# wenyuqing/panacea

Hardware: AMD Instinct MI355X
Metric: denoising steps/s (6-view x 8-frame 256x512) (higher is better)
Workload: dtype f16; 1 GPU; BASELINE config 3: Panacea+ stage-2 UNet+ControlNet, CFG 2 x 8 frames, 6 views, latent 32x384, hint 256x3072, Euler/LegacyDDPM 50-step schedule; precision=precise: split(stream,gn_stt,ff_out,stem,gn_head,gnt)+e4m3-lo, parallelism=single, graph=False, streams=2, hoisted_step_invariants=False, fused_step_tail=True

## Files before the change

### include/panacea_hip.h

```cpp
#ifndef PANACEA_HIP_H
#define PANACEA_HIP_H

#include <stdint.h>

#ifdef __cplusplus
extern "C" {
#endif

#define PNC_OK 0
#define PNC_EINVAL (-1)
#define PNC_EALIGN (-2)
#define PNC_EABI (-3)

const char* pnc_version(void);
#define PNC_ABI_VERSION 8
int pnc_abi_version(void);
const char* pnc_build_digest(void);

enum {
    PNC_OPT_GEMM_TAIL_SPLIT = 0,
    PNC_OPT_GEMM_TILE = 1,
    PNC_OPT_ATTN_VARIANT = 2,
    PNC_OPT_ATTN_DMA = 3,
    PNC_OPT_GEMM_FUSE_LN = 4,
    PNC_OPT_GEMM_GROUP_M = 5,
    PNC_OPT_STENCIL_TILES = 6,
    PNC_OPT_GEMM_PERSIST = 7,
    PNC_OPT_ATTN_DEFER_MAX = 8,
    PNC_OPT_GEMM_GN_STATS = 9,
    PNC_OPT_GEMM_STAGGER = 10,
    PNC_OPT_ATTN_SUM_TRIGGER = 11,
    PNC_OPT_COUNT = 12
};
int pnc_set_option(int option, int value);

enum { PNC_A_PLAIN = 0, PNC_A_CONV3X3 = 1, PNC_A_CONV1D_T = 2 };
enum { PNC_LO_F16 = 0, PNC_LO_E4M3 = 1 };
enum { PNC_ACT_NONE = 0, PNC_ACT_SILU = 1, PNC_ACT_GELU = 2  };

typedef struct PncGemmParams {
    const void* A;
    const void* W;
    int32_t M, N, K;
    int32_t lda;
    int32_t a_mode;
// ... 44 lines not shown
    int32_t groups;
    int32_t heads;
    int32_t H, W, views;
    int32_t kvH, kvW, kv_views;
    int32_t kv_rows_per_group;
    int32_t q_per_kv;
    int32_t kv_valid;
    int32_t nseg[8];
    int32_t seg[8][2];
    float scale;
    int32_t causal;
    const void* k_halo[2];
    const void* vt_halo[2];
} PncAttnParams;

int pnc_attn_views_f16(const PncAttnParams* p, void* stream);

int pnc_attn_temporal_f16(const void* q, int ldq, const void* k, int ldk,
                          const void* v, int ldv, void* o, int ldo,
                          int B, int T, int Npix, int heads, float scale, void* stream);

typedef struct PncAttnSplitParams {
    int32_t struct_bytes;
    PncAttnParams a;
    const void* q_lo;
    const void* k_lo;
    const void* v_lo;
    void* o_lo;
} PncAttnSplitParams;
int pnc_attn_views_split_f16(const PncAttnSplitParams* p, void* stream);
int pnc_attn_temporal_split_f16(const void* q, const void* q_lo, int ldq, const void* k, const void* k_lo, int ldk,
                                const void* v, const void* v_lo, int ldv, void* o, void* o_lo, int ldo,
                                int B, int T, int Npix, int heads, float scale, void* stream);

int pnc_groupnorm_stats(const float* x, int ldx, int F, int Npix, int C,
                        int pix_per_chunk, float* partial, void* stream);
int pnc_groupnorm_apply(const float* x, int ldx, int F, int Npix, int C,
                        int pix_per_chunk, const float* partial,
                        const float* gamma, const float* beta, float eps, int silu,
                        void* y16, int ldy, void* y16_lo, int lo_fmt, int n_records, void* stream);
int pnc_groupnorm_combine(const float* in, int parts, int F, int nchunk, float* out, void* stream);
int pnc_groupnorm_temporal_silu(const float* x, int B, int T, int Npix, int C,
                                const float* gamma, const float* beta, float eps,
                                void* y16, void* y16_lo, int lo_fmt, void* stream);
int pnc_groupnorm_temporal_part(const float* x, int B, int T, int Npix, int C,
                                const float* gamma, const float* beta, float eps,
                                float* stats, int mode, int T_total,
                                void* y16, void* y16_lo, int lo_fmt, int t_pad, void* stream);
int pnc_layernorm(const float* x, int ldx, int M, int C,
                  const float* gamma, const float* beta, float eps,
                  void* y16, int ldy, void* y16_lo, void* stream);

int pnc_linear_smallm(const float* a, int lda, const void* W, const float* bias,
                      float* out, int ldo, int M, int N, int K, int silu_in, int silu_out,
                      void* stream);
#define PNC_SMALLM_MAX_SEGS 64
int pnc_linear_smallm_segments(const float* a, int lda, const void* W, const float* bias, float* out, int M,
                               int m0, int Mtot, int N, int K, const int32_t* seg_start, int nseg, int silu_in,
                               int silu_out, void* stream);
int pnc_timestep_embedding(const int64_t* t, int F, int dim, const float* freqs,
                           float* out, void* stream);
int pnc_nchw_to_tokens_f16(const float* a, int C1, const float* a_scale, int a_frames, const float* b, int C2,
                           int F, int Npix, int Cpad, void* out16, void* out16_lo, void* stream);
int pnc_cfg_euler_step(const float* eps_tok, int ld, int T, int Npix, int C, int cfg, float scale,
                       const float* x, const float* c_out, const float* sigma, const float* sigma_next, float* x_next,
                       void* stream);
// ... 44 lines not shown
```

### panacea_amd/build.py

```python
from __future__ import annotations

import hashlib
import os
import shutil
import subprocess
import sys
from pathlib import Path

PKG = Path(__file__).resolve().parent
ROOT = PKG.parent
CSRC = PKG / "csrc"
LIBDIR = PKG / "lib"
LIB = LIBDIR / "libpanacea_hip.so"
SOURCES = ["gemm.hip", "gemm_plain.hip", "gemm_conv3x3.hip", "gemm_stencil_tile.hip", "gemm_conv1d.hip", "attn.hip", "attn_split.hip", "norm.hip", "misc.hip"]
HEADERS = [CSRC / "common.h", CSRC / "gemm_kernel.h", ROOT / "include" / "panacea_hip.h"]
FLAGS = ["--offload-arch=gfx950", "-O3", "-std=c++17", "-fPIC", "-Wall", "-Wno-unused-function",
         "-I", str(ROOT / "include"), "-I", str(CSRC)]


def _hipcc() -> str:
    for cand in (os.environ.get("HIPCC"), shutil.which("hipcc"), "/opt/rocm/bin/hipcc"):
        if cand and Path(cand).exists():
            return cand
    raise RuntimeError("hipcc not found (expected /opt/rocm/bin/hipcc)")


def _digest() -> str:
    h = hashlib.sha256()
    for f in [CSRC / s for s in SOURCES] + HEADERS:
        h.update(f.read_bytes())
    h.update(" ".join(f.replace(str(ROOT), "<root>") for f in FLAGS).encode())
    return h.hexdigest()


def library_digest(lib: Path = LIB):
    try:
        blob = Path(lib).read_bytes()
    except OSError:
        return None
    i = blob.find(_DIGEST_MARK)
    if i < 0:
        return None
    j = blob.find(b"\0", i)
    return blob[i + len(_DIGEST_MARK):j].decode(errors="replace")


_DIGEST_MARK = b"pnc-build-digest:"
# ... 40 lines not shown
```

### panacea_amd/csrc/attn.hip

```cpp
#include "common.h"
#include <stdlib.h>

namespace {

constexpr int KT = 64;

__device__ __forceinline__ int kperm(int i) { return 16 * ((i >> 2) & 1) + 4 * (i >> 3) + (i & 3); }

__device__ __attribute__((aligned(16))) half_t g_attn_zero_chunk[8];

template <int NW, int QB, bool DMA>
__global__ __launch_bounds__(64 * NW, (NW == 4 && QB == 2 && DMA) ? 2 : 1) void attn_views_kernel(const PncAttnParams p, const int wv_shift,
                                                                                          const float defer_thr, const int dma_mode,
                                                                                          const float sum_lim) {
    constexpr int QT = NW * QB * 32;
    constexpr int ROWS_PER_IT = NW * 8;
    constexpr int ST_IT = 64 / ROWS_PER_IT;
    constexpr int NST = DMA ? 3 : 2;
    __shared__ __attribute__((aligned(16))) char smem[NST * 2 * KT * 128];
    const half_t* __restrict__ Q = reinterpret_cast<const half_t*>(p.q);
    const half_t* __restrict__ K = reinterpret_cast<const half_t*>(p.k);
    const half_t* __restrict__ VT = reinterpret_cast<const half_t*>(p.vt);
    half_t* __restrict__ O = reinterpret_cast<half_t*>(p.o);
    auto seg_view = [&](int id, const half_t*& Kb, const half_t*& Vb) -> int {
// ... 534 lines not shown
extern "C" int pnc_attn_views_f16(const PncAttnParams* pp, void* stream) {
    if (!pp) return PNC_EINVAL;
    const PncAttnParams& p = *pp;
    if (!p.q || !p.k || !p.vt || !p.o) return PNC_EINVAL;
    if (p.views < 1 || p.views > 8 || p.kv_views < 1 || p.kv_views > 8) return PNC_EINVAL;
    if (p.W % p.views || p.kvW % p.kv_views) return PNC_EINVAL;
    const int kvWv = p.kvW / p.kv_views;
    (void)kvWv;
    if (p.ldq % 8 || p.ldk % 8 || p.ldo % 4) return PNC_EALIGN;
    if (((uintptr_t)p.q | (uintptr_t)p.k) & 15) return PNC_EALIGN;
    if ((uintptr_t)p.vt & 15) return PNC_EALIGN;
    if ((uintptr_t)p.o & 7) return PNC_EALIGN;
    if (p.q_per_kv < 1 || p.groups < 1 || p.heads < 1) return PNC_EINVAL;
    if (p.kv_valid < 1 || p.kv_valid > p.kvH * kvWv) return PNC_EINVAL;
    if (p.causal != 0 && p.causal != 1) return PNC_EINVAL;
    for (int v = 0; v < p.views; ++v) {
        if (p.nseg[v] < 1 || p.nseg[v] > 2) return PNC_EINVAL;
        for (int s = 0; s < p.nseg[v]; ++s) {
            const int id = p.seg[v][s];
            if (id == -1 || id == p.kv_views) {
                const int side = id < 0 ? 0 : 1;
                if (!p.k_halo[side] || !p.vt_halo[side]) return PNC_EINVAL;
                if (((uintptr_t)p.k_halo[side] | (uintptr_t)p.vt_halo[side]) & 15) return PNC_EALIGN;
            } else if (id < 0 || id > p.kv_views) {
                return PNC_EINVAL;
            }
        }
    }
    const int Nq = p.H * (p.W / p.views);
    const int force = pnc_get_option(PNC_OPT_ATTN_VARIANT);
    const int kv_keys = p.kv_valid * 2;
    {
        const bool text_ok = p.views == 1 && p.kv_views == 1 && p.nseg[0] == 1 && p.seg[0][0] == 0 && !p.causal && p.kvH * p.kvW <= 96 &&
                             p.kv_valid > 64 && p.kv_valid <= 96 && (p.ldvt & 7) == 0 && (p.vt_gstride & 7) == 0 && (p.ldk & 7) == 0;
        constexpr int HG = 5;
        const int nhg = (p.heads + HG - 1) / HG;
        const long nwg = (long)((Nq + 127) / 128) * nhg * p.groups;
        const bool big_enough = (long)((Nq + 127) / 128) * nhg >= 16;
        const int dopt = pnc_get_option(PNC_OPT_ATTN_DMA);
        if (text_ok && (force == 43 || (force == 0 && big_enough)) && (dopt & 3) != 0 && !(dopt & 4)) {
            const dim3 grid((unsigned)nwg);
            hipLaunchKernelGGL((attn_text_kernel<HG>), grid, dim3(256), 0, reinterpret_cast<hipStream_t>(stream), p, nhg);
            return pnc_launch_status();
        }
    }
    const int big = force == 1 ? 82 : 42;
    const int variant = force >= 41 ? force : (kv_keys <= 256 ? (Nq >= 256 ? 42 : 41) : (Nq >= 512 ? big : (Nq >= 256 ? 81 : 41)));
    hipStream_t st = reinterpret_cast<hipStream_t>(stream);
    const int dma_mode = pnc_get_option(PNC_OPT_ATTN_DMA) & 3;
    const bool dma = ((kvWv & 7) == 0) && ((p.kvW & 7) == 0) && ((p.ldvt & 7) == 0) && ((p.vt_gstride & 7) == 0) && dma_mode != 0;
    int wv_shift = -1;
    if (kvWv > 0 && (kvWv & (kvWv - 1)) == 0) { wv_shift = 0; while ((1 << wv_shift) < kvWv) ++wv_shift; }
    int dopt = pnc_get_option(PNC_OPT_ATTN_DEFER_MAX);
    const float defer_thr = (float)(dopt < 0 ? 0 : (dopt > 14 ? 14 : dopt));
    const int sopt = pnc_get_option(PNC_OPT_ATTN_SUM_TRIGGER);
    const float sum_lim = sopt <= 0 ? 0.0f : ldexpf(1.0f, sopt > 14 ? 14 : sopt);
#define PNC_ATTN_LAUNCH(NW_, QB_, QTILE_)                                                                         \
    do {                                                                                                          \
        dim3 grid(((Nq + (QTILE_) - 1) / (QTILE_)) * p.views * p.groups * p.heads);                               \
        if (dma) hipLaunchKernelGGL((attn_views_kernel<NW_, QB_, true>), grid, dim3(64 * NW_), 0, st, p, wv_shift, defer_thr, dma_mode, sum_lim);  \
        else hipLaunchKernelGGL((attn_views_kernel<NW_, QB_, false>), grid, dim3(64 * NW_), 0, st, p, wv_shift, defer_thr, dma_mode, sum_lim);   \
    } while (0)
    if (variant == 42) PNC_ATTN_LAUNCH(4, 2, 256);
    else if (variant == 82) PNC_ATTN_LAUNCH(8, 2, 512);
    else if (variant == 81) PNC_ATTN_LAUNCH(8, 1, 256);
    else PNC_ATTN_LAUNCH(4, 1, 128);
// ... 22 lines not shown
```

### panacea_amd/hip.py

```python
from __future__ import annotations

import ctypes as C
import re
from pathlib import Path
from typing import Optional

import torch

PKG = Path(__file__).resolve().parent
LIB_PATH = PKG / "lib" / "libpanacea_hip.so"
HEADER = PKG.parent / "include" / "panacea_hip.h"

A_PLAIN, A_CONV3X3, A_CONV1D_T = 0, 1, 2
ACT_NONE, ACT_SILU, ACT_GELU = 0, 1, 2
ABI_VERSION = 8
LO_F16, LO_E4M3 = 0, 1
LO_DTYPE = {LO_F16: torch.float16, LO_E4M3: torch.uint8}


def lo_fmt(t: Optional[torch.Tensor]) -> int:
    if t is None or t.dtype == torch.float16:
        return LO_F16
    if t.dtype == torch.uint8:
        return LO_E4M3
# ... 29 lines not shown
        ("A_lo", C.c_void_p), ("out16_lo", C.c_void_p),
        ("ldw", C.c_int32), ("ln_eps", C.c_float),
        ("ln_gamma", C.c_void_p), ("ln_beta", C.c_void_p), ("ln_out16", C.c_void_p),
        ("ldln", C.c_int32), ("a_lo_fmt", C.c_int32),
        ("out_lo_fmt", C.c_int32), ("ldw_lo", C.c_int32),
        ("W_lo", C.c_void_p), ("w_lo_exp", C.c_int32), ("t_halo", C.c_int32),
        ("x_halo_off", C.c_int64), ("gn_part", C.c_void_p),
    ]


class AttnParams(C.Structure):
    _fields_ = [
        ("q", C.c_void_p), ("ldq", C.c_int32),
        ("k", C.c_void_p), ("ldk", C.c_int32),
        ("vt", C.c_void_p), ("ldvt", C.c_int32), ("vt_gstride", C.c_int64),
        ("o", C.c_void_p), ("ldo", C.c_int32),
        ("groups", C.c_int32), ("heads", C.c_int32),
        ("H", C.c_int32), ("W", C.c_int32), ("views", C.c_int32),
        ("kvH", C.c_int32), ("kvW", C.c_int32), ("kv_views", C.c_int32),
        ("kv_rows_per_group", C.c_int32), ("q_per_kv", C.c_int32), ("kv_valid", C.c_int32),
        ("nseg", C.c_int32 * 8), ("seg", (C.c_int32 * 2) * 8),
        ("scale", C.c_float), ("causal", C.c_int32),
        ("k_halo", C.c_void_p * 2), ("vt_halo", C.c_void_p * 2),
    ]


class AttnSplitParams(C.Structure):
    _fields_ = [
        ("struct_bytes", C.c_int32), ("a", AttnParams),
        ("q_lo", C.c_void_p), ("k_lo", C.c_void_p), ("v_lo", C.c_void_p), ("o_lo", C.c_void_p),
    ]


class SamplerStepParams(C.Structure):
    _fields_ = [
        ("struct_bytes", C.c_int32), ("mode", C.c_int32),
        ("eps_tok", C.c_void_p), ("ld", C.c_int32), ("T", C.c_int32), ("Npix", C.c_int32), ("C", C.c_int32),
        ("cfg", C.c_int32), ("scale", C.c_float),
        ("x", C.c_void_p), ("c_out", C.c_void_p), ("x0", C.c_void_p), ("aux", C.c_void_p),
        ("hist", C.c_void_p * 4), ("n_hist", C.c_int32), ("s_noise", C.c_float), ("noise", C.c_void_p),
        ("v", C.c_void_p * 6), ("out", C.c_void_p), ("out_aux", C.c_void_p),
    ]


SAMPLER_HEUN1, SAMPLER_HEUN2, SAMPLER_EULER_A, SAMPLER_DPM2S_1, SAMPLER_DPM2S_2, SAMPLER_DPM2M, SAMPLER_LMS = range(7)


_P, _I, _L, _F = C.c_void_p, C.c_int, C.c_int64, C.c_float
_SIGNATURES = {
    "pnc_version": (C.c_char_p, []),
    "pnc_abi_version": (_I, []),
    "pnc_build_digest": (C.c_char_p, []),
    "pnc_set_option": (_I, [_I, _I]),
    "pnc_gemm_f16": (_I, [C.POINTER(GemmParams), _P]),
    "pnc_gemm_workspace_floats": (_L, [C.POINTER(GemmParams)]),
    "pnc_gemm_fuses_layernorm": (_I, [C.POINTER(GemmParams)]),
    "pnc_attn_views_f16": (_I, [C.POINTER(AttnParams), _P]),
    "pnc_attn_views_split_f16": (_I, [C.POINTER(AttnSplitParams), _P]),
    "pnc_attn_temporal_split_f16": (_I, [_P, _P, _I, _P, _P, _I, _P, _P, _I, _P, _P, _I, _I, _I, _I, _I, _F, _P]),
    "pnc_softmax_rows_f16": (_I, [_P, _L, _I, _I, _F, _I, _I, _P, _L, _P]),
    "pnc_attn_temporal_f16": (_I, [_P, _I, _P, _I, _P, _I, _P, _I, _I, _I, _I, _I, _F, _P]),
    "pnc_groupnorm_stats": (_I, [_P, _I, _I, _I, _I, _I, _P, _P]),
    "pnc_groupnorm_apply": (_I, [_P, _I, _I, _I, _I, _I, _P, _P, _P, _F, _I, _P, _I, _P, _I, _I, _P]),
    "pnc_groupnorm_combine": (_I, [_P, _I, _I, _I, _P, _P]),
    "pnc_groupnorm_temporal_part": (_I, [_P, _I, _I, _I, _I, _P, _P, _F, _P, _I, _I, _P, _P, _I, _I, _P]),
    "pnc_groupnorm_temporal_silu": (_I, [_P, _I, _I, _I, _I, _P, _P, _F, _P, _P, _I, _P]),
    "pnc_layernorm": (_I, [_P, _I, _I, _I, _P, _P, _F, _P, _I, _P, _P]),
    "pnc_linear_smallm": (_I, [_P, _I, _P, _P, _P, _I, _I, _I, _I, _I, _I, _P]),
    "pnc_linear_smallm_segments": (_I, [_P, _I, _P, _P, _P, _I, _I, _I, _I, _I, _P, _I, _I, _I, _P]),
    "pnc_timestep_embedding": (_I, [_P, _I, _I, _P, _P, _P]),
    "pnc_nchw_to_tokens_f16": (_I, [_P, _I, _P, _I, _P, _I, _I, _I, _I, _P, _P, _P]),
    "pnc_cfg_euler_step": (_I, [_P, _I, _I, _I, _I, _I, _F, _P, _P, _P, _P, _P, _P]),
    "pnc_cfg_sampler_step": (_I, [C.POINTER(SamplerStepParams), _P]),
    "pnc_tokens_to_nchw_f32": (_I, [_P, _I, _I, _I, _I, _P, _P]),
    "pnc_concat_add": (_I, [_P, _I, _P, _P, _I, _L, _P, _P, _P, _I, _P]),
    "pnc_concat_add_stats": (_I, [_P, _I, _P, _P, _I, _I, _I, _I, _P, _P, _P, _I, _P, _P]),
    "pnc_add_f32": (_I, [_P, _P, _L, _P, _P, _P, _I, _P]),
    "pnc_cast_f16": (_I, [_P, _L, _P, _P, _I, _P]),
    "pnc_range_monitor_collect": (_I, [_P, _P]),
}

_lib = None


def header_symbols() -> list[str]:
    txt = HEADER.read_text()
    txt = re.sub(r"/\*.*?\*/", "", txt, flags=re.S)
    return sorted(set(re.findall(r"\b(pnc_[a-z0-9_]+)\s*\(", txt)))


def load():
# ... 12 lines not shown
        lib = C.CDLL(str(LIB_PATH))
    except OSError as e:
        raise HipLibraryError(f"cannot load {LIB_PATH}: {e}") from e
    if not os.environ.get("PANACEA_HIP_LIB"):
        from . import build as _build
        try:
            lib.pnc_build_digest.restype = C.c_char_p
            have = lib.pnc_build_digest().decode()
        except AttributeError:
            have = "(a library older than pnc_build_digest)"
        if _build.CSRC.exists() and have != _build._digest():
            raise HipLibraryError(f"{LIB_PATH} was built from other sources ({have[:12]}) than panacea_amd/csrc holds now "
                                  f"({_build._digest()[:12]}); rebuild it with `python -m panacea_amd.build`")
    for name, (res, args) in _SIGNATURES.items():
        try:
            fn = getattr(lib, name)
        except AttributeError as e:
            raise HipLibraryError(f"{LIB_PATH} does not export {name}; rebuild the extension") from e
        fn.restype = res
        fn.argtypes = args
    if lib.pnc_abi_version() != ABI_VERSION:
        raise HipLibraryError(f"{LIB_PATH} implements C-ABI version {lib.pnc_abi_version()}, this binding needs "
                              f"{ABI_VERSION}; rebuild the extension (`python -m panacea_amd.build --force`)")
    _lib = lib
    return lib


OPT_GEMM_TAIL_SPLIT, OPT_GEMM_TILE, OPT_ATTN_VARIANT, OPT_ATTN_DMA, OPT_GEMM_FUSE_LN, OPT_GEMM_GROUP_M, OPT_STENCIL_TILES = 0, 1, 2, 3, 4, 5, 6
OPT_GEMM_PERSIST = 7
OPT_ATTN_DEFER_MAX = 8
OPT_GEMM_GN_STATS = 9
OPT_GEMM_STAGGER = 10
OPT_ATTN_SUM_TRIGGER = 11


def build_digest() -> str:
    return load().pnc_build_digest().decode()


def set_option(option: int, value: int) -> int:
    if not 0 <= option <= OPT_ATTN_SUM_TRIGGER:
        raise PncError(f"unknown library option {option}")
    return load().pnc_set_option(option, value)


CU_MASK_PATTERNS = {
    "even-odd": ([0x55555555] * 8, [0xAAAAAAAA] * 8),
    "nibbles": ([0x0F0F0F0F] * 8, [0xF0F0F0F0] * 8),
    "halves": ([0xFFFFFFFF] * 4 + [0] * 4, [0] * 4 + [0xFFFFFFFF] * 4),
}


def masked_stream(words) -> "torch.cuda.Stream":
    rt = None
    for line in open("/proc/self/maps"):
        if "libamdhip64" in line:
            rt = C.CDLL(line.split()[-1])
            break
    if rt is None:
        raise PncError("the HIP runtime is not loaded")
    rt.hipExtStreamCreateWithCUMask.argtypes = [C.POINTER(C.c_void_p), C.c_uint32, C.POINTER(C.c_uint32)]
    rt.hipExtStreamCreateWithCUMask.restype = C.c_int
    st = C.c_void_p()
    arr = (C.c_uint32 * len(words))(*words)
    rc = rt.hipExtStreamCreateWithCUMask(C.byref(st), C.c_uint32(len(words)), arr)
    if rc != 0:
# ... 122 lines not shown
    _check(_timed(fam, 2.0 * M * N * K, 0.0, lib.pnc_gemm_f16, C.byref(p), _stream()), "pnc_gemm_f16")
    if trailing_ln:
        layernorm(out32, ldc32, M, N, ln_gamma, ln_beta, ln_eps, ln_out16, ldln)


def _attn_params(p, q, ldq, k, ldk, vt, ldvt, vt_gstride, o, ldo, groups, heads, H, W, views, kvH, kvW, kv_views,
                 kv_rows_per_group, q_per_kv, kv_valid, segs, scale, causal):
    p.q, p.ldq, p.k, p.ldk = _ptr(q), ldq, _ptr(k), ldk
    p.vt, p.ldvt, p.vt_gstride, p.o, p.ldo = _ptr(vt), ldvt, vt_gstride, _ptr(o), ldo
    p.groups, p.heads, p.H, p.W, p.views = groups, heads, H, W, views
    p.kvH, p.kvW, p.kv_views = kvH, kvW, kv_views
    p.kv_rows_per_group, p.q_per_kv, p.kv_valid = kv_rows_per_group, q_per_kv, kv_valid
    for v, s in enumerate(segs):
        p.nseg[v] = len(s)
        for j, u in enumerate(s):
            p.seg[v][j] = u
    p.scale, p.causal = scale, int(causal)


def attn_views(q, ldq, k, ldk, vt, ldvt, vt_gstride, o, ldo, *, groups, heads, H, W, views,
               kvH, kvW, kv_views, kv_rows_per_group, q_per_kv, kv_valid, segs, scale, causal=False, k_halo=None, vt_halo=None):
    p = AttnParams()
    if k_halo is not None:
        for i in range(2):
            p.k_halo[i], p.vt_halo[i] = _ptr(k_halo[i]), _ptr(vt_halo[i])
    _attn_params(p, q, ldq, k, ldk, vt, ldvt, vt_gstride, o, ldo, groups, heads, H, W, views, kvH, kvW, kv_views,
                 kv_rows_per_group, q_per_kv, kv_valid, segs, scale, causal)
    nq = H * (W // views)
    nkeys = sum(len(sv) for sv in segs) * kv_valid
    _check(_timed("attn_views", 4.0 * groups * heads * nq * nkeys * 64, 0.0, load().pnc_attn_views_f16,
                  C.byref(p), _stream()), "pnc_attn_views_f16")


def attn_views_split(q, q_lo, ldq, k, k_lo, ldk, v, v_lo, ldv, o, o_lo, ldo, *, groups, heads, H, W, views, kvH, kvW, kv_views,
                     kv_rows_per_group, q_per_kv, kv_valid, segs, scale):
    f16 = torch.float16
    sp = AttnSplitParams()
    sp.struct_bytes = C.sizeof(AttnSplitParams)
    _attn_params(sp.a, q, ldq, k, ldk, v, ldv, 0, o, ldo, groups, heads, H, W, views, kvH, kvW, kv_views, kv_rows_per_group,
                 q_per_kv, kv_valid, segs, scale, False)
    sp.q_lo, sp.k_lo = _ptr(q_lo, f16, "q_lo"), _ptr(k_lo, f16, "k_lo")
    sp.v_lo, sp.o_lo = _ptr(v_lo, f16, "v_lo"), _ptr(o_lo, f16, "o_lo")
    nq = H * (W // views)
    nkeys = sum(len(sv) for sv in segs) * kv_valid
    _check(_timed("attn_views_split", 12.0 * groups * heads * nq * nkeys * 64, 0.0, load().pnc_attn_views_split_f16,
                  C.byref(sp), _stream()), "pnc_attn_views_split_f16")


def attn_temporal_split(q, q_lo, ldq, k, k_lo, ldk, v, v_lo, ldv, o, o_lo, ldo, *, B, T, Npix, heads, scale):
    f16 = torch.float16
    nb = 16.0 * B * T * Npix * heads * 64
    _check(_timed("attn_temporal_split", 0.0, nb, load().pnc_attn_temporal_split_f16,
                  _ptr(q, f16, "q"), _ptr(q_lo, f16, "q_lo"), ldq, _ptr(k, f16, "k"), _ptr(k_lo, f16, "k_lo"), ldk,
                  _ptr(v, f16, "v"), _ptr(v_lo, f16, "v_lo"), ldv, _ptr(o, f16, "o"), _ptr(o_lo, f16, "o_lo"), ldo,
                  B, T, Npix, heads, scale, _stream()), "pnc_attn_temporal_split_f16")


def softmax_rows(s32, lds, M, N, scale, p16, ldp, causal=False, n_valid=0):
    _check(_timed("softmax_rows", 0.0, 6.0 * M * N, load().pnc_softmax_rows_f16, _ptr(s32), lds, M, N, scale, int(causal),
                  n_valid, _ptr(p16), ldp, _stream()), "pnc_softmax_rows_f16")


def attn_temporal(q, ldq, k, ldk, v, ldv, o, ldo, *, B, T, Npix, heads, scale):
    nb = 8.0 * B * T * Npix * heads * 64
    _check(_timed("attn_temporal", 0.0, nb, load().pnc_attn_temporal_f16, _ptr(q), ldq, _ptr(k), ldk, _ptr(v), ldv,
                  _ptr(o), ldo, B, T, Npix, heads, scale, _stream()), "pnc_attn_temporal_f16")
# ... 122 lines not shown
```

### panacea_amd/nn/attention.py

```python
from __future__ import annotations

import math
from typing import Optional

import torch
from torch import nn

from .. import engine as E
from ..engine import Act, Packable, Runtime

HEAD_DIM = 64
INTRA_SEGS = [[0], [1], [2], [3], [4], [5]]
INTER_SEGS = [[5, 1], [0, 2], [1, 3], [2, 4], [3, 5], [4]]


def exists(v):
    return v is not None


def default(v, d):
    return v if v is not None else (d() if callable(d) else d)


def Normalize(in_channels):
# ... 93 lines not shown

    def _text_kv(self, rt: Runtime):
        hit = rt.text_kv.get(id(self))
        if hit is not None:
            return hit
        pk = self.packed()
        C, D, rows = self.inner_dim, rt.ctx16.shape[1], rt.B * E.TEXT_PAD
        if rt.prec.kv_text:
            kv, kv_lo = rt.empty((rows, 2 * C), torch.float16), rt.lo_plane((rows, 2 * C), "kv_text")
            if "wkv" not in pk:
                pk["wkv"] = torch.cat([pk["wk"], pk["wv"]]).contiguous()
            rt.be.gemm(rt.ctx16, pk["wkv"], M=rows, N=2 * C, K=D, lda=D, out16=kv, ldc16=2 * C, out16_lo=kv_lo, a16_lo=rt.ctx16_lo)
            f, fl = kv.view(-1), kv_lo.view(-1)
            return f, fl, f[C:], fl[C:], 2 * C
        k = rt.empty((rows, C), torch.float16)
        vt = rt.empty((rt.B, C, E.TEXT_PAD), torch.float16)
        rt.be.gemm(rt.ctx16, pk["wk"], M=rows, N=C, K=D, lda=D, out16=k, ldc16=C)
        rt.be.gemm(rt.ctx16, pk["wv"], M=rows, N=C, K=D, lda=D, out16t=vt, ldt=E.TEXT_PAD, t_rows=E.TEXT_PAD,
                   t_gstride=C * E.TEXT_PAD, n_split=0)
        return k, C, vt, E.TEXT_PAD, C * E.TEXT_PAD

    def _run_text(self, rt: Runtime, x16, F, H, W, res32, out32, ln=None, x16_lo=None):
        pk = self.packed()
        C, M = self.inner_dim, F * H * W
        if rt.prec.q_text:
            q, q_lo = rt.empty((M, C), torch.float16), rt.lo_plane((M, C), "q_text")
            rt.be.gemm(x16, pk["wq"], M=M, N=C, K=self.query_dim, lda=self.query_dim, out16=q, ldc16=C, out16_lo=q_lo, a16_lo=x16_lo)
            k, k_lo, v, v_lo, ld = self._text_kv(rt)
            o, o_lo = rt.empty((M, C), torch.float16), rt.lo_plane((M, C), "attn_o")
            rt.be.attn_views_split(q, q_lo, C, k, k_lo, ld, v, v_lo, ld, o, o_lo, C, groups=F, heads=self.heads, H=H, W=W,
                                   views=1, kvH=1, kvW=E.TEXT_PAD, kv_views=1, kv_rows_per_group=E.TEXT_PAD, q_per_kv=F // rt.B,
                                   kv_valid=rt.n_text, segs=[[0]], scale=self.scale)
            return self._out_proj(rt, o, o_lo, M, C, res32, out32, ln)
        q = rt.empty((M, C), torch.float16)
        rt.be.gemm(x16, pk["wq"], M=M, N=C, K=self.query_dim, lda=self.query_dim, out16=q, ldc16=C)
        k, ldk, vt, ldvt, vt_gs = self._text_kv(rt)
        o = rt.empty((M, C), torch.float16)
        rt.be.attn_views(q, C, k, ldk, vt, ldvt, vt_gs, o, C, groups=F, heads=self.heads, H=H, W=W,
                         views=1, kvH=1, kvW=E.TEXT_PAD, kv_views=1, kv_rows_per_group=E.TEXT_PAD,
                         q_per_kv=F // rt.B, kv_valid=rt.n_text, segs=[[0]], scale=self.scale)
        lnkw, y16 = _ln_kwargs(rt, ln, M, self.query_dim)
        rt.be.gemm(o, pk["wo"], M=M, N=self.query_dim, K=C, lda=C, bias=pk["bo"], res1=res32,
                   ldr1=self.query_dim, out32=out32, ldc32=self.query_dim, **lnkw)
        return y16, None

    def _out_proj(self, rt: Runtime, o, o_lo, M, C, res32, out32, ln):
        pk = self.packed()
        rt.be.gemm(o, pk["wo"], M=M, N=self.query_dim, K=C, lda=C, bias=pk["bo"], res1=res32, ldr1=self.query_dim, out32=out32,
                   ldc32=self.query_dim, a16_lo=o_lo)
        return _ln_after(rt, ln, out32, M, self.query_dim, None)

    def _qkv_split(self, rt: Runtime, x16, x16_lo, M):
        pk = self.packed()
        C = self.inner_dim
        qkv, qkv_lo = rt.empty((M, 3 * C), torch.float16), rt.lo_plane((M, 3 * C), "qkv")
        rt.be.gemm(x16, pk["wqkv"], M=M, N=3 * C, K=self.query_dim, lda=self.query_dim, out16=qkv, ldc16=3 * C, out16_lo=qkv_lo,
                   a16_lo=x16_lo)
        return qkv.view(-1), qkv_lo.view(-1)

    def _run_views(self, rt: Runtime, x16, F, H, W, segs, res32, out32, ln=None, x16_lo=None):
        pk = self.packed()
        C, N = self.inner_dim, H * W
        M = F * N
        vs = rt.vshard if len(segs) == E.ViewShard.VIEWS else None
        views = vs.n_local if vs is not None else len(segs)
        if W % views:
            raise ValueError(f"grid width {W} is not divisible into {views} views")
        if rt.prec.qkv:
            if rt.vshard is not None:
                raise ValueError("the precise-wide operand policy does not run view-sharded")
            f, fl = self._qkv_split(rt, x16, x16_lo, M)
            o, o_lo = rt.empty((M, C), torch.float16), rt.lo_plane((M, C), "attn_o")
            rt.be.attn_views_split(f, fl, 3 * C, f[C:], fl[C:], 3 * C, f[2 * C:], fl[2 * C:], 3 * C, o, o_lo, C, groups=F,
# ... 327 lines not shown
```

Measured before the change: 6.549 steps/s.

## Fuse text cross-attention Q projection into attention kernel

Adds a HIP kernel that computes the query projection (x·Wq) per head inside the text cross-attention kernel, keeping Q in registers instead of writing and re-reading a Q tensor. It is enabled by default only when the query width is 320. When x fits, a variant keeps the x fragments in registers and streams only Wq through LDS. This removes one GEMM launch and the Q round trip to memory, at the cost of recomputing nothing but with more LDS per workgroup and a narrower applicability check. The existing text attention kernel also gains an extra alignment guard on the key count.

Result: no change. 6.579 steps/s (median of 6 runs) (+0.5%).

```diff
diff --git a/include/panacea_hip.h b/include/panacea_hip.h
--- a/include/panacea_hip.h
+++ b/include/panacea_hip.h
@@ -11,6 +11,7 @@
 #define PNC_EINVAL (-1)
 #define PNC_EALIGN (-2)
 #define PNC_EABI (-3)
+#define PNC_UNHANDLED 1
 
 const char* pnc_version(void);
 #define PNC_ABI_VERSION 8
@@ -121,6 +122,16 @@
 int pnc_attn_temporal_split_f16(const void* q, const void* q_lo, int ldq, const void* k, const void* k_lo, int ldk,
                                 const void* v, const void* v_lo, int ldv, void* o, void* o_lo, int ldo,
                                 int B, int T, int Npix, int heads, float scale, void* stream);
+
+#define PNC_TEXT_PROJ_MAX_CQ 320
+typedef struct PncAttnTextProjParams {
+    int32_t struct_bytes;
+    PncAttnParams a;
+    const void* x;  int32_t ldx;
+    const void* wq; int32_t ldw;
+    int32_t cq;
+} PncAttnTextProjParams;
+int pnc_attn_text_proj_f16(const PncAttnTextProjParams* p, void* stream);
 
 int pnc_groupnorm_stats(const float* x, int ldx, int F, int Npix, int C,
                         int pix_per_chunk, float* partial, void* stream);
diff --git a/panacea_amd/build.py b/panacea_amd/build.py
--- a/panacea_amd/build.py
+++ b/panacea_amd/build.py
@@ -12,7 +12,7 @@
 CSRC = PKG / "csrc"
 LIBDIR = PKG / "lib"
 LIB = LIBDIR / "libpanacea_hip.so"
-SOURCES = ["gemm.hip", "gemm_plain.hip", "gemm_conv3x3.hip", "gemm_stencil_tile.hip", "gemm_conv1d.hip", "attn.hip", "attn_split.hip", "norm.hip", "misc.hip"]
+SOURCES = ["gemm.hip", "gemm_plain.hip", "gemm_conv3x3.hip", "gemm_stencil_tile.hip", "gemm_conv1d.hip", "attn.hip", "attn_text_proj.hip", "attn_split.hip", "norm.hip", "misc.hip"]
 HEADERS = [CSRC / "common.h", CSRC / "gemm_kernel.h", ROOT / "include" / "panacea_hip.h"]
 FLAGS = ["--offload-arch=gfx950", "-O3", "-std=c++17", "-fPIC", "-Wall", "-Wno-unused-function",
          "-I", str(ROOT / "include"), "-I", str(CSRC)]
diff --git a/panacea_amd/csrc/attn.hip b/panacea_amd/csrc/attn.hip
--- a/panacea_amd/csrc/attn.hip
+++ b/panacea_amd/csrc/attn.hip
@@ -590,6 +590,7 @@
     const int kv_keys = p.kv_valid * 2;
     {
         const bool text_ok = p.views == 1 && p.kv_views == 1 && p.nseg[0] == 1 && p.seg[0][0] == 0 && !p.causal && p.kvH * p.kvW <= 96 &&
+                             ((p.kvH * p.kvW) & 7) == 0 &&
                              p.kv_valid > 64 && p.kv_valid <= 96 && (p.ldvt & 7) == 0 && (p.vt_gstride & 7) == 0 && (p.ldk & 7) == 0;
         constexpr int HG = 5;
         const int nhg = (p.heads + HG - 1) / HG;
diff --git a/panacea_amd/csrc/attn_text_proj.hip b/panacea_amd/csrc/attn_text_proj.hip
--- /dev/null
+++ b/panacea_amd/csrc/attn_text_proj.hip
@@ -0,0 +1,336 @@
+#include "common.h"
+#include <atomic>
+
+namespace {
+
+__device__ __forceinline__ int kperm(int i) { return 16 * ((i >> 2) & 1) + 4 * (i >> 3) + (i & 3); }
+
+__device__ __attribute__((aligned(16))) half_t g_textproj_zero_chunk[8];
+
+constexpr int KROWS = 96;
+constexpr int KV_BYTES = KROWS * 128 + 2 * 64 * 128;
+constexpr int X_BYTES = 128 * 128, W_BYTES = 64 * 128;
+constexpr int PSTAGE = X_BYTES + W_BYTES;
+constexpr int LDS_BYTES = KV_BYTES + 2 * PSTAGE;
+
+__device__ __forceinline__ void attend_head(const f32x16 (&acc)[2], const char* skv, const f32x16& init2, const f32x16& zero16, const float sc,
+                                            const int krow_lds, const int frow, const int grp, half_t* orow, const bool qok,
+                                            const bool vec16) {
+    half8v qf[4];
+#pragma unroll
+    for (int dh = 0; dh < 2; ++dh)
+#pragma unroll
+        for (int rp = 0; rp < 2; ++rp) {
+            half4v he, ho;
+#pragma unroll
+            for (int q = 0; q < 4; ++q) {
+                he[q] = (half_t)acc[dh][(2 * rp) * 4 + q];
+                ho[q] = (half_t)acc[dh][(2 * rp + 1) * 4 + q];
+            }
+            union { half4v h; int2 i; } snd, rcv;
+            snd.h = grp ? he : ho;
+            rcv.i.x = __shfl_xor(snd.i.x, 32, 64);
+            rcv.i.y = __shfl_xor(snd.i.y, 32, 64);
+            half8v q8;
+#pragma unroll
+            for (int q = 0; q < 4; ++q) {
+                q8[q] = grp ? rcv.h[q] : he[q];
+                q8[4 + q] = grp ? ho[q] : rcv.h[q];
+            }
+            qf[dh * 2 + rp] = q8;
+        }
+    const char* sk = skv;
+    const char* sv = skv + KROWS * 128;
+    f32x16 s[3];
+#pragma unroll
+    for (int kb = 0; kb < 3; ++kb) {
+#pragma unroll
+        for (int ds = 0; ds < 4; ++ds) {
+            const half8v kf = *reinterpret_cast<const half8v*>(sk + lds_off128(kb * 32 + krow_lds, ds * 2 + grp));
+            s[kb] = __builtin_amdgcn_mfma_f32_32x32x16_f16(kf, qf[ds], ds == 0 ? (kb == 2 ? init2 : zero16) : s[kb], 0, 0, 0);
+        }
+    }
+    float tmax = -1e30f;
+#pragma unroll
+    for (int kb = 0; kb < 3; ++kb)
+#pragma unroll
+        for (int r = 0; r < 16; ++r) tmax = fmaxf(tmax, s[kb][r]);
+    const float m = fmaxf(tmax, __shfl_xor(tmax, 32, 64)) * sc;
+    half8v pf[3][2];
+    float psum = 0.0f;
+#pragma unroll
+    for (int kb = 0; kb < 3; ++kb)
+#pragma unroll
+        for (int r = 0; r < 16; ++r) {
+            const float pv = __builtin_amdgcn_exp2f(fmaf(s[kb][r], sc, -m));
+            psum += pv;
+            pf[kb][r >> 3][r & 7] = (half_t)pv;
+        }
+    const float ltot = psum + __shfl_xor(psum, 32, 64);
+    f32x16 oacc[2] = {zero16, zero16};
+#pragma unroll
+    for (int dh = 0; dh < 2; ++dh)
+#pragma unroll
+        for (int kb = 0; kb < 3; ++kb) {
+#pragma unroll
+            for (int ss = 0; ss < 2; ++ss) {
+                const half8v vf = *reinterpret_cast<const half8v*>(sv + (kb >> 1) * 8192 + lds_off128(dh * 32 + frow, (kb & 1) * 4 + grp * 2 + ss));
+                oacc[dh] = __builtin_amdgcn_mfma_f32_32x32x16_f16(vf, pf[kb][ss], oacc[dh], 0, 0, 0);
+            }
+        }
+    const float inv = ltot > 0.0f ? 1.0f / ltot : 0.0f;
+#pragma unroll
+    for (int dh = 0; dh < 2; ++dh)
+#pragma unroll
+        for (int rp = 0; rp < 2; ++rp) {
+            half4v he, ho;
+#pragma unroll
+            for (int q = 0; q < 4; ++q) {
+                he[q] = (half_t)(oacc[dh][(2 * rp) * 4 + q] * inv);
+                ho[q] = (half_t)(oacc[dh][(2 * rp + 1) * 4 + q] * inv);
+            }
+            if (vec16) {
+                union { half4v h; int2 i; } snd, rcv;
+                snd.h = grp ? he : ho;
+                rcv.i.x = __shfl_xor(snd.i.x, 32, 64);
+                rcv.i.y = __shfl_xor(snd.i.y, 32, 64);
+                half8v o8;
+#pragma unroll
+                for (int q = 0; q < 4; ++q) {
+                    o8[q] = grp ? rcv.h[q] : he[q];
+                    o8[4 + q] = grp ? ho[q] : rcv.h[q];
+                }
+                if (qok) *reinterpret_cast<half8v*>(orow + dh * 32 + 8 * (2 * rp + grp)) = o8;
+            } else if (qok) {
+                *reinterpret_cast<half4v*>(orow + dh * 32 + 8 * (2 * rp) + 4 * grp) = he;
+                *reinterpret_cast<half4v*>(orow + dh * 32 + 8 * (2 * rp + 1) + 4 * grp) = ho;
+            }
+        }
+}
+
+template <int HG>
+__global__ __launch_bounds__(256, 2) void attn_text_proj_kernel(const PncAttnParams p, const half_t* __restrict__ X, const int ldx,
+                                                                const half_t* __restrict__ Wq, const int ldw, const int Cq,
+                                                                const int nhg) {
+    extern __shared__ __attribute__((aligned(16))) char smem[];
+    char* const skv = smem;
+    char* const sproj = smem + KV_BYTES;
+    const half_t* __restrict__ K = reinterpret_cast<const half_t*>(p.k);
+    const half_t* __restrict__ VT = reinterpret_cast<const half_t*>(p.vt);
+    half_t* __restrict__ O = reinterpret_cast<half_t*>(p.o);
+    const int tid = threadIdx.x, lane = tid & 63;
+    const int wave = __builtin_amdgcn_readfirstlane(tid >> 6);
+    const int Nq = p.H * p.W, nqt = (Nq + 127) >> 7;
+    const int Nkv = p.kvH * p.kvW;
+    const int item = blockIdx.x;
+    const int hg = item % nhg, qt = (item / nhg) % nqt, g = item / (nhg * nqt);
+    const int kvg = g / p.q_per_kv;
+    const int h0 = hg * HG, nh = min(HG, p.heads - h0);
+    const int grp = lane >> 5, frow = lane & 31;
+    const int ql = qt * 128 + wave * 32 + frow;
+    const bool qok = ql < Nq;
+    const int64_t qrow = (int64_t)g * Nq + (qok ? ql : Nq - 1);
+    const int nkt = Cq >> 6;
+
+    const int sr = tid >> 3, sc8 = (tid & 7) ^ ((sr >> 1) & 7);
+    const half_t* xsrc[4];
+#pragma unroll
+    for (int i = 0; i < 4; ++i) {
+        const int r = qt * 128 + sr + 32 * i;
+        xsrc[i] = X + ((int64_t)g * Nq + min(r, Nq - 1)) * ldx + sc8 * 8;
+    }
+    const half_t* const wsrc0 = Wq + (int64_t)(h0 * 64 + sr) * ldw + sc8 * 8;
+    auto dma_proj = [&](int hh, int kt, int stage) {
+        char* sx = sproj + stage * PSTAGE + wave * 1024;
+        char* sw = sx + X_BYTES;
+#pragma unroll
+        for (int i = 0; i < 4; ++i) glds16(xsrc[i] + kt * 64, sx + i * 4096);
+        const half_t* w = wsrc0 + (int64_t)hh * 64 * ldw + kt * 64;
+#pragma unroll
+        for (int i = 0; i < 2; ++i) glds16(w + (int64_t)(32 * i) * ldw, sw + i * 4096);
+    };
+    auto dma_kv = [&](int hh) {
+        const int hc = (h0 + hh) * 64;
+        char* sk = skv + wave * 1024;
+#pragma unroll
+        for (int i = 0; i < KROWS / 32; ++i) {
+            const int key = sr + 32 * i;
+            const half_t* src = key < Nkv ? K + ((int64_t)kvg * p.kv_rows_per_group + key) * p.ldk + hc + sc8 * 8 : g_textproj_zero_chunk;
+            glds16(src, sk + i * 4096);
+        }
+        char* sv = skv + KROWS * 128 + wave * 1024;
+#pragma unroll
+        for (int j = 0; j < 2; ++j)
+#pragma unroll
+            for (int i = 0; i < 2; ++i) {
+                const int d = sr + 32 * i, kc = j * 64 + sc8 * 8;
+                const half_t* src = kc < Nkv ? VT + (int64_t)kvg * p.vt_gstride + (int64_t)(hc + d) * p.ldvt + kc : g_textproj_zero_chunk;
+                glds16(src, sv + j * 8192 + i * 4096);
+            }
+    };
+
+    const float sc = p.scale * 1.44269504088896340736f;
+    const int krow_lds = kperm(frow);
+    f32x16 init2;
+#pragma unroll
+    for (int r = 0; r < 16; ++r) init2[r] = (64 + grp * 16 + r >= p.kv_valid) ? -1e30f : 0.0f;
+    const f32x16 zero16 = {0.0f, 0.0f, 0.0f, 0.0f, 0.0f, 0.0f, 0.0f, 0.0f, 0.0f, 0.0f, 0.0f, 0.0f, 0.0f, 0.0f, 0.0f, 0.0f};
+    const bool vec16 = ((p.ldo & 7) == 0) && (((uintptr_t)p.o & 15) == 0);
+
+    dma_proj(0, 0, 0);
+    int T = 0;
+    for (int hh = 0; hh < nh; ++hh) {
+        f32x16 acc[2] = {zero16, zero16};
+        for (int kt = 0; kt < nkt; ++kt, ++T) {
+            asm volatile("s_waitcnt vmcnt(0)" ::: "memory");
+            __builtin_amdgcn_s_barrier();
+            if (kt + 1 < nkt) dma_proj(hh, kt + 1, (T + 1) & 1);
+            else if (hh + 1 < nh) dma_proj(hh + 1, 0, (T + 1) & 1);
+            if (kt == 0) dma_kv(hh);
+            const char* sx = sproj + (T & 1) * PSTAGE;
+            const char* sw = sx + X_BYTES;
+#pragma unroll
+            for (int ks = 0; ks < 4; ++ks) {
+                const half8v xf = *reinterpret_cast<const half8v*>(sx + lds_off128(wave * 32 + frow, ks * 2 + grp));
+#pragma unroll
+                for (int dh = 0; dh < 2; ++dh) {
+                    const half8v wf = *reinterpret_cast<const half8v*>(sw + lds_off128(dh * 32 + frow, ks * 2 + grp));
+                    acc[dh] = __builtin_amdgcn_mfma_f32_32x32x16_f16(wf, xf, acc[dh], 0, 0, 0);
+                }
+            }
+        }
+        attend_head(acc, skv, init2, zero16, sc, krow_lds, frow, grp, O + qrow * p.ldo + (h0 + hh) * 64, qok, vec16);
+    }
+}
+
+template <int HG, int NKT>
+__global__ __launch_bounds__(256, 2) void attn_text_proj_xreg_kernel(const PncAttnParams p, const half_t* __restrict__ X, const int ldx,
+                                                                     const half_t* __restrict__ Wq, const int ldw, const int nhg) {
+    extern __shared__ __attribute__((aligned(16))) char smem[];
+    char* const skv = smem;
+    char* const swq = smem + KV_BYTES;
+    const half_t* __restrict__ K = reinterpret_cast<const half_t*>(p.k);
+    const half_t* __restrict__ VT = reinterpret_cast<const half_t*>(p.vt);
+    half_t* __restrict__ O = reinterpret_cast<half_t*>(p.o);
+    const int tid = threadIdx.x, lane = tid & 63;
+    const int wave = __builtin_amdgcn_readfirstlane(tid >> 6);
+    const int Nq = p.H * p.W, nqt = (Nq + 127) >> 7;
+    const int Nkv = p.kvH * p.kvW;
+    const int item = blockIdx.x;
+    const int hg = item % nhg, qt = (item / nhg) % nqt, g = item / (nhg * nqt);
+    const int kvg = g / p.q_per_kv;
+    const int h0 = hg * HG, nh = min(HG, p.heads - h0);
+    const int grp = lane >> 5, frow = lane & 31;
+    const int ql = qt * 128 + wave * 32 + frow;
+    const bool qok = ql < Nq;
+    const int64_t qrow = (int64_t)g * Nq + (qok ? ql : Nq - 1);
+    half8v xf[NKT * 4];
+#pragma unroll
+    for (int ks = 0; ks < NKT * 4; ++ks) xf[ks] = *reinterpret_cast<const half8v*>(X + qrow * ldx + ks * 16 + grp * 8);
+    const int sr = tid >> 3, sc8 = (tid & 7) ^ ((sr >> 1) & 7);
+    const half_t* const wsrc0 = Wq + (int64_t)(h0 * 64 + sr) * ldw + sc8 * 8;
+    auto dma_w = [&](int hh) {
+        const half_t* w = wsrc0 + (int64_t)hh * 64 * ldw;
+        char* sw = swq + wave * 1024;
+#pragma unroll
+        for (int kt = 0; kt < NKT; ++kt)
+#pragma unroll
+            for (int i = 0; i < 2; ++i) glds16(w + (int64_t)(32 * i) * ldw + kt * 64, sw + kt * W_BYTES + i * 4096);
+    };
+    auto dma_kv = [&](int hh) {
+        const int hc = (h0 + hh) * 64;
+        char* sk = skv + wave * 1024;
+#pragma unroll
+        for (int i = 0; i < KROWS / 32; ++i) {
+            const int key = sr + 32 * i;
+            const half_t* src = key < Nkv ? K + ((int64_t)kvg * p.kv_rows_per_group + key) * p.ldk + hc + sc8 * 8 : g_textproj_zero_chunk;
+            glds16(src, sk + i * 4096);
+        }
+        char* sv = skv + KROWS * 128 + wave * 1024;
+#pragma unroll
+        for (int j = 0; j < 2; ++j)
+#pragma unroll
+            for (int i = 0; i < 2; ++i) {
+                const int d = sr + 32 * i, kc = j * 64 + sc8 * 8;
+                const half_t* src = kc < Nkv ? VT + (int64_t)kvg * p.vt_gstride + (int64_t)(hc + d) * p.ldvt + kc : g_textproj_zero_chunk;
+                glds16(src, sv + j * 8192 + i * 4096);
+            }
+    };
+    const float sc = p.scale * 1.44269504088896340736f;
+    const int krow_lds = kperm(frow);
+    f32x16 init2;
+#pragma unroll
+    for (int r = 0; r < 16; ++r) init2[r] = (64 + grp * 16 + r >= p.kv_valid) ? -1e30f : 0.0f;
+    const f32x16 zero16 = {0.0f, 0.0f, 0.0f, 0.0f, 0.0f, 0.0f, 0.0f, 0.0f, 0.0f, 0.0f, 0.0f, 0.0f, 0.0f, 0.0f, 0.0f, 0.0f};
+    const bool vec16 = ((p.ldo & 7) == 0) && (((uintptr_t)p.o & 15) == 0);
+
+    dma_w(0);
+    for (int hh = 0; hh < nh; ++hh) {
+        asm volatile("s_waitcnt vmcnt(0)" ::: "memory");
+        __builtin_amdgcn_s_barrier();
+        dma_kv(hh);
+        f32x16 acc[2] = {zero16, zero16};
+#pragma unroll
+        for (int ks = 0; ks < NKT * 4; ++ks)
+#pragma unroll
+            for (int dh = 0; dh < 2; ++dh) {
+                const half8v wf = *reinterpret_cast<const half8v*>(swq + (ks >> 2) * W_BYTES + lds_off128(dh * 32 + frow, (ks & 3) * 2 + grp));
+                acc[dh] = __builtin_amdgcn_mfma_f32_32x32x16_f16(wf, xf[ks], acc[dh], 0, 0, 0);
+            }
+        asm volatile("s_waitcnt vmcnt(0) lgkmcnt(0)" ::: "memory");
+        __builtin_amdgcn_s_barrier();
+        if (hh + 1 < nh) dma_w(hh + 1);
+        attend_head(acc, skv, init2, zero16, sc, krow_lds, frow, grp, O + qrow * p.ldo + (h0 + hh) * 64, qok, vec16);
+    }
+}
+
+}
+
+static bool textproj_default_on(int Cq) { return Cq == PNC_TEXT_PROJ_MAX_CQ; }
+
+extern "C" int pnc_attn_text_proj_f16(const PncAttnTextProjParams* pp, void* stream) {
+    if (!pp) return PNC_EINVAL;
+    if (pp->struct_bytes != (int32_t)sizeof(PncAttnTextProjParams)) return PNC_EABI;
+    const PncAttnParams& p = pp->a;
+    if (!pp->x || !pp->wq || !p.k || !p.vt || !p.o) return PNC_EINVAL;
+    if (p.views < 1 || p.kv_views < 1 || p.q_per_kv < 1 || p.groups < 1 || p.heads < 1 || p.H < 1 || p.W < 1) return PNC_EINVAL;
+    if (p.kv_valid < 1 || p.kv_valid > p.kvH * p.kvW) return PNC_EINVAL;
+    if (pp->cq < 1 || pp->ldx < pp->cq || pp->ldw < pp->cq) return PNC_EINVAL;
+    if (p.ldk % 8 || p.ldo % 4) return PNC_EALIGN;
+    if (((uintptr_t)p.k | (uintptr_t)p.vt) & 15) return PNC_EALIGN;
+    if ((uintptr_t)p.o & 7) return PNC_EALIGN;
+    const int dopt = pnc_get_option(PNC_OPT_ATTN_DMA);
+    if ((dopt & 8) || (dopt & 4) || (dopt & 3) == 0) return PNC_UNHANDLED;
+    const int force = pnc_get_option(PNC_OPT_ATTN_VARIANT);
+    if (force != 0 && force != 43) return PNC_UNHANDLED;
+    const int Nkv = p.kvH * p.kvW;
+    const bool text_ok = p.views == 1 && p.kv_views == 1 && p.nseg[0] == 1 && p.seg[0][0] == 0 && !p.causal && Nkv <= 96 && (Nkv & 7) == 0 &&
+                         p.kv_valid > 64 && p.kv_valid <= 96 && (p.ldvt & 7) == 0 && (p.vt_gstride & 7) == 0 && (p.ldk & 7) == 0;
+    const bool proj_ok = (pp->cq & 63) == 0 && pp->cq >= 128 && (pp->ldx & 7) == 0 && (pp->ldw & 7) == 0 &&
+                         (((uintptr_t)pp->x | (uintptr_t)pp->wq) & 15) == 0;
+    if (!text_ok || !proj_ok) return PNC_UNHANDLED;
+    constexpr int HG = 5;
+    const int Nq = p.H * p.W;
+    const int nhg = (p.heads + HG - 1) / HG;
+    const bool big_enough = (long)((Nq + 127) / 128) * nhg >= 16;
+    if (!(force == 43 || big_enough)) return PNC_UNHANDLED;
+    if (!(dopt & 16) && !textproj_default_on(pp->cq)) return PNC_UNHANDLED;
+    static std::atomic<unsigned char> attr_done[64];
+    int dev = 0;
+    (void)hipGetDevice(&dev);
+    constexpr int NKT_REG = PNC_TEXT_PROJ_MAX_CQ / 64, LDS_XREG = KV_BYTES + NKT_REG * W_BYTES;
+    if (!attr_done[dev & 63].load(std::memory_order_acquire)) {
+        (void)hipFuncSetAttribute(reinterpret_cast<const void*>(attn_text_proj_kernel<HG>), hipFuncAttributeMaxDynamicSharedMemorySize, LDS_BYTES);
+        (void)hipFuncSetAttribute(reinterpret_cast<const void*>(attn_text_proj_xreg_kernel<HG, NKT_REG>),
+                                  hipFuncAttributeMaxDynamicSharedMemorySize, LDS_XREG);
+        attr_done[dev & 63].store(1, std::memory_order_release);
+    }
+    const long nwg = (long)((Nq + 127) / 128) * nhg * p.groups;
+    if (pp->cq == NKT_REG * 64)
+        hipLaunchKernelGGL((attn_text_proj_xreg_kernel<HG, NKT_REG>), dim3((unsigned)nwg), dim3(256), LDS_XREG, reinterpret_cast<hipStream_t>(stream),
+                           p, reinterpret_cast<const half_t*>(pp->x), pp->ldx, reinterpret_cast<const half_t*>(pp->wq), pp->ldw, nhg);
+    else
+        hipLaunchKernelGGL((attn_text_proj_kernel<HG>), dim3((unsigned)nwg), dim3(256), LDS_BYTES, reinterpret_cast<hipStream_t>(stream), p,
+                           reinterpret_cast<const half_t*>(pp->x), pp->ldx, reinterpret_cast<const half_t*>(pp->wq), pp->ldw, pp->cq, nhg);
+    return pnc_launch_status();
+}
diff --git a/panacea_amd/hip.py b/panacea_amd/hip.py
--- a/panacea_amd/hip.py
+++ b/panacea_amd/hip.py
@@ -85,6 +85,13 @@
     ]
 
 
+class AttnTextProjParams(C.Structure):
+    _fields_ = [
+        ("struct_bytes", C.c_int32), ("a", AttnParams),
+        ("x", C.c_void_p), ("ldx", C.c_int32), ("wq", C.c_void_p), ("ldw", C.c_int32), ("cq", C.c_int32),
+    ]
+
+
 class SamplerStepParams(C.Structure):
     _fields_ = [
         ("struct_bytes", C.c_int32), ("mode", C.c_int32),
@@ -110,6 +117,7 @@
     "pnc_gemm_fuses_layernorm": (_I, [C.POINTER(GemmParams)]),
     "pnc_attn_views_f16": (_I, [C.POINTER(AttnParams), _P]),
     "pnc_attn_views_split_f16": (_I, [C.POINTER(AttnSplitParams), _P]),
+    "pnc_attn_text_proj_f16": (_I, [C.POINTER(AttnTextProjParams), _P]),
     "pnc_attn_temporal_split_f16": (_I, [_P, _P, _I, _P, _P, _I, _P, _P, _I, _P, _P, _I, _I, _I, _I, _I, _F, _P]),
     "pnc_softmax_rows_f16": (_I, [_P, _L, _I, _I, _F, _I, _I, _P, _L, _P]),
     "pnc_attn_temporal_f16": (_I, [_P, _I, _P, _I, _P, _I, _P, _I, _I, _I, _I, _I, _F, _P]),
@@ -188,6 +196,8 @@
 OPT_GEMM_GN_STATS = 9
 OPT_GEMM_STAGGER = 10
 OPT_ATTN_SUM_TRIGGER = 11
+ATTN_DMA_NO_TEXT_KERNEL, ATTN_DMA_NO_TEXT_FUSE_Q, ATTN_DMA_TEXT_FUSE_Q_ALL = 4, 8, 16
+UNHANDLED = 1
 
 
 def build_digest() -> str:
@@ -376,6 +386,31 @@
                   C.byref(p), _stream()), "pnc_attn_views_f16")
 
 
+def attn_text_proj(x16, ldx, wq, cq, k, ldk, vt, ldvt, vt_gstride, o, ldo, *, groups, heads, H, W, kvH, kvW, kv_rows_per_group,
+                   q_per_kv, kv_valid, scale) -> bool:
+    f16 = torch.float16
+    tp = AttnTextProjParams()
+    tp.struct_bytes = C.sizeof(AttnTextProjParams)
+    _attn_params(tp.a, None, 0, k, ldk, vt, ldvt, vt_gstride, o, ldo, groups, heads, H, W, 1, kvH, kvW, 1, kv_rows_per_group,
+                 q_per_kv, kv_valid, [[0]], scale, False)
+    tp.x, tp.ldx, tp.wq, tp.ldw, tp.cq = _ptr(x16, f16, "x16"), ldx, _ptr(wq, f16, "wq"), wq.shape[-1], cq
+    fn, st = load().pnc_attn_text_proj_f16, _stream()
+    if _PROF is None:
+        rc = fn(C.byref(tp), st)
+    else:
+        e0, e1 = torch.cuda.Event(enable_timing=True), torch.cuda.Event(enable_timing=True)
+        e0.record()
+        rc = fn(C.byref(tp), st)
+        e1.record()
+        if rc == 0:
+            M, Cc = groups * H * W, heads * 64
+            _PROF.records.append(("attn_text_proj", e0, e1, 4.0 * M * heads * kv_valid * 64 + 2.0 * M * Cc * cq, 0.0))
+    if rc == UNHANDLED:
+        return False
+    _check(rc, "pnc_attn_text_proj_f16")
+    return True
+
+
 def attn_views_split(q, q_lo, ldq, k, k_lo, ldk, v, v_lo, ldv, o, o_lo, ldo, *, groups, heads, H, W, views, kvH, kvW, kv_views,
                      kv_rows_per_group, q_per_kv, kv_valid, segs, scale):
     f16 = torch.float16
diff --git a/panacea_amd/nn/attention.py b/panacea_amd/nn/attention.py
--- a/panacea_amd/nn/attention.py
+++ b/panacea_amd/nn/attention.py
@@ -149,13 +149,17 @@
                                    views=1, kvH=1, kvW=E.TEXT_PAD, kv_views=1, kv_rows_per_group=E.TEXT_PAD, q_per_kv=F // rt.B,
                                    kv_valid=rt.n_text, segs=[[0]], scale=self.scale)
             return self._out_proj(rt, o, o_lo, M, C, res32, out32, ln)
-        q = rt.empty((M, C), torch.float16)
-        rt.be.gemm(x16, pk["wq"], M=M, N=C, K=self.query_dim, lda=self.query_dim, out16=q, ldc16=C)
         k, ldk, vt, ldvt, vt_gs = self._text_kv(rt)
         o = rt.empty((M, C), torch.float16)
-        rt.be.attn_views(q, C, k, ldk, vt, ldvt, vt_gs, o, C, groups=F, heads=self.heads, H=H, W=W,
-                         views=1, kvH=1, kvW=E.TEXT_PAD, kv_views=1, kv_rows_per_group=E.TEXT_PAD,
-                         q_per_kv=F // rt.B, kv_valid=rt.n_text, segs=[[0]], scale=self.scale)
+        fused = getattr(rt.be, "attn_text_proj", None)
+        if fused is None or not fused(x16, self.query_dim, pk["wq"], self.query_dim, k, ldk, vt, ldvt, vt_gs, o, C, groups=F,
+                                      heads=self.heads, H=H, W=W, kvH=1, kvW=E.TEXT_PAD, kv_rows_per_group=E.TEXT_PAD,
+                                      q_per_kv=F // rt.B, kv_valid=rt.n_text, scale=self.scale):
+            q = rt.empty((M, C), torch.float16)
+            rt.be.gemm(x16, pk["wq"], M=M, N=C, K=self.query_dim, lda=self.query_dim, out16=q, ldc16=C)
+            rt.be.attn_views(q, C, k, ldk, vt, ldvt, vt_gs, o, C, groups=F, heads=self.heads, H=H, W=W,
+                             views=1, kvH=1, kvW=E.TEXT_PAD, kv_views=1, kv_rows_per_group=E.TEXT_PAD,
+                             q_per_kv=F // rt.B, kv_valid=rt.n_text, segs=[[0]], scale=self.scale)
         lnkw, y16 = _ln_kwargs(rt, ln, M, self.query_dim)
         rt.be.gemm(o, pk["wo"], M=M, N=self.query_dim, K=C, lda=C, bias=pk["bo"], res1=res32,
                    ldr1=self.query_dim, out32=out32, ldc32=self.query_dim, **lnkw)
```
